# huggingface/optimum-quanto

Hardware: AMD Instinct MI355X
Metric: QLinear GEMM TFLOP/s (bf16 x int8 qbytes_mm) (higher is better)
Workload: dtype bf16; 1 GPU; bf16 x int8 qbytes_mm, per-channel scale, (M,K,N)=(4096,4096,4096); M=4096, K=4096, N=4096, weight_buffers_rotated=1, launch=hipGraph replay of the K steps, parallelism=replicas x1 (no data-path collective)

## Files before the change

### include/quanto_hip.h

```cpp
#ifndef QUANTO_HIP_H_
#define QUANTO_HIP_H_

#include <stddef.h>
#include <stdint.h>

#ifdef __cplusplus
extern "C" {
#endif

#define QUANTO_HIP_ABI_VERSION 1

typedef enum {
  QUANTO_HIP_OK = 0,
  QUANTO_HIP_EINVAL = -1,
  QUANTO_HIP_ENOTSUP = -2,
  QUANTO_HIP_ELAUNCH = -3,
  QUANTO_HIP_EALIGN = -4
} quanto_hip_status;

typedef enum {
  QUANTO_HIP_F32 = 0,
  QUANTO_HIP_F16 = 1,
  QUANTO_HIP_BF16 = 2,
  QUANTO_HIP_I8 = 3,
// ... 59 lines not shown
int64_t quanto_hip_qbits_mm_workspace_size(int64_t M, int64_t N, int64_t K, int bits, int group_size, int dtype,
                                           int kernel);
int quanto_hip_qbits_mm_pick(int64_t M, int64_t N, int64_t K, int bits, int group_size, int dtype);
int quanto_hip_qbits_mm_plan(int64_t M, int64_t N, int64_t K, int bits, int group_size, int dtype, int kernel, int* kernel_out,
                             int64_t* workspace_bytes_out);

int quanto_hip_qbytes_mm(const void* a, const void* b, const void* scales, const void* bias, void* y,
                         int64_t M, int64_t N, int64_t K, int a_dtype, int b_dtype, int out_dtype, int kernel,
                         void* stream);

int quanto_hip_qbytes_mm_multi_ws(const void* a, int count, const void* const* b, const void* const* scales,
                                  const void* const* bias, void* const* y, const int64_t* N, int64_t M, int64_t K, int a_dtype,
                                  int b_dtype, int out_dtype, void* workspace, size_t workspace_bytes, void* stream);
int quanto_hip_qbytes_mm_multi_plan(int count, const int64_t* N, int64_t M, int64_t K, int a_dtype, int b_dtype, int out_dtype,
                                    int* kernel_out, int64_t* workspace_bytes_out);

int quanto_hip_qbytes_mm_ws(const void* a, const void* b, const void* scales, const void* bias, void* y,
                            int64_t M, int64_t N, int64_t K, int a_dtype, int b_dtype, int out_dtype, int kernel,
                            void* workspace, size_t workspace_bytes, void* stream);
int64_t quanto_hip_qbytes_mm_workspace_size(int64_t M, int64_t N, int64_t K, int a_dtype, int b_dtype, int out_dtype, int kernel);
int quanto_hip_qbytes_mm_pick(int64_t M, int64_t N, int64_t K, int a_dtype, int b_dtype, int out_dtype);
int quanto_hip_qbytes_mm_plan(int64_t M, int64_t N, int64_t K, int a_dtype, int b_dtype, int out_dtype, int kernel, int* kernel_out,
                              int64_t* workspace_bytes_out);

int quanto_hip_qbytes_mm_q_ws(const void* a, const void* b, const void* scales, const void* bias, const void* out_scale, void* yq,
                              int64_t M, int64_t N, int64_t K, int a_dtype, int b_dtype, int mid_dtype, int kernel,
                              void* workspace, size_t workspace_bytes, void* stream);
int quanto_hip_qbytes_mm_q_plan(int64_t M, int64_t N, int64_t K, int a_dtype, int b_dtype, int mid_dtype, int kernel, int* kernel_out,
                                int64_t* workspace_bytes_out);

enum quanto_hip_scale_mode { QUANTO_HIP_SCALE_PER_TENSOR = 0, QUANTO_HIP_SCALE_AXIS_FIRST = 1, QUANTO_HIP_SCALE_AXIS_LAST = 2 };
int quanto_hip_quantize_symmetric(const void* base, const void* scale, void* out, int64_t numel, int64_t inner,
                                  int scale_mode, int in_dtype, int out_dtype, void* stream);

int quanto_hip_dequantize_symmetric(const void* q, const void* scale, void* out, int64_t numel, int q_dtype, int out_dtype, void* stream);

int quanto_hip_quantize_affine(const void* base, const void* scale, const void* shift, uint8_t* out, int64_t N, int64_t K,
                               int bits, int group_size, int dtype, int shift_dtype, void* stream);

int quanto_hip_quantize_affine_packed(const void* base, const void* scale, const void* shift, uint8_t* packed, int64_t N, int64_t K,
                                      int bits, int group_size, int dtype, int shift_dtype, void* stream);

int quanto_hip_pack(const uint8_t* unpacked, uint8_t* packed, int64_t rows, int64_t cols, int bits, void* stream);

int quanto_hip_qbits_mm_a8(const void* a, const void* a_scale, const uint8_t* packed, const void* scale, const void* shift, const void* bias, void* y,
                           int64_t M, int64_t N, int64_t K, int bits, int group_size, int a_dtype, int dtype, int shift_dtype, void* workspace,
// ... 57 lines not shown
```

### optimum_quanto_amd/csrc/c_api.hip

```cpp
#include "qh_conv.h"

namespace qh {

static thread_local const char* g_last_kernel = "";
void set_last_kernel(const char* name) { g_last_kernel = name; }

int launch_status() { return hipGetLastError() == hipSuccess ? QUANTO_HIP_OK : QUANTO_HIP_ELAUNCH; }

int unpack_dispatch(const uint8_t*, uint8_t*, int64_t, int, hipStream_t);
int dequantize_qbits_dispatch(const uint8_t*, const void*, const void*, void*, const PackedGeom&, int, bool, hipStream_t);
int qbytes_mm_naive(const void*, const void*, const void*, const void*, void*, int64_t, int64_t, int64_t, int, int, int, hipStream_t);
int qbits_mm_naive(const void*, const uint8_t*, const void*, const void*, const void*, void*, int64_t, const PackedGeom&, int, bool,
                   hipStream_t);
bool qbits_gemv_supported(int64_t, const PackedGeom&, int);
int qbits_mm_gemv(const void*, const uint8_t*, const void*, const void*, const void*, void*, int64_t, const PackedGeom&, int, bool,
                  hipStream_t);
int qbits_mm_gemv_multi(const void*, int, const uint8_t* const*, const void* const*, const void* const*, const void* const*, void* const*,
                        const int64_t*, int64_t, int64_t, int, bool, hipStream_t);
bool qbytes_gemv_supported(int64_t, int64_t, int64_t, int, int, int);
int qbytes_mm_gemv(const void*, const void*, const void*, const void*, void*, int64_t, int64_t, int64_t, int, int, int, hipStream_t);
bool qbytes_mfma_supported(int64_t, int64_t, int64_t, int, int, int);
int qbytes_mm_mfma(const void*, const void*, const void*, const void*, void*, int64_t, int64_t, int64_t, int, int, int, hipStream_t);
bool qbytes_mfma_large_supported(int64_t, int64_t, int64_t, int, int, int);
int qbytes_mm_mfma_large(const void*, const void*, const void*, const void*, void*, int64_t, int64_t, int64_t, int, int, int, void*, size_t, hipStream_t);
size_t qbytes_mfma_large_workspace(int64_t, int64_t, int64_t);
int quantize_symmetric(const void*, const void*, void*, int64_t, int64_t, int, int, int, hipStream_t);
int dequantize_symmetric(const void*, const void*, void*, int64_t, int, int, hipStream_t);
int quantize_affine(const void*, const void*, const void*, void*, int64_t, int64_t, int, int, bool, hipStream_t);
int quantize_affine_packed(const void*, const void*, const void*, void*, int64_t, int64_t, int, int, bool, hipStream_t);
int pack_weights(const uint8_t*, uint8_t*, int64_t, int64_t, int, hipStream_t);
bool qbits_conv2d_supported(const ConvGeom&, const PackedGeom&, int);
int qbits_conv2d_mfma(const void*, const uint8_t*, const void*, const void*, const void*, void*, const ConvGeom&, const PackedGeom&, int, bool, void*, size_t,
                      hipStream_t);
size_t conv2d_workspace(int64_t, int64_t, int64_t);
int qbytes_conv2d_depthwise(const void*, const void*, const void*, const void*, void*, const ConvGeom&, int, int, int, hipStream_t, bool* strip);
size_t conv2d_dense_weight_bytes(int64_t, int64_t);
bool conv2d_rows_eligible(const ConvGeom&);
int qdense_conv2d_rows(const void*, const void*, const void*, void*, const ConvGeom&, int, void*, size_t, hipStream_t);
int qbytes_conv2d_a8_kind(int, int, int);
size_t conv2d_a8_workspace(int64_t, int64_t, int64_t);
int qbytes_conv2d_a8(const void*, const void*, const void*, const void*, const void*, const void*, void*, const ConvGeom&, int, int, int, void*, size_t,
                     hipStream_t, int*);
int qbytes_conv2d_mfma(const void*, const void*, const void*, const void*, void*, const ConvGeom&, int, int, int, void*, size_t, hipStream_t, bool* rows);
int qbytes_mm_gemv_multi(const void*, int, const void* const*, const void* const*, const void* const*, void* const*, const int64_t*, int64_t,
                         int64_t, int, int, hipStream_t);
bool qbytes_skinny_multi_supported(int, const int64_t*, int64_t, int64_t, int, int, int);
size_t qbytes_skinny_multi_workspace(int, const int64_t*, int64_t, int64_t);
int qbytes_mm_skinny_multi(const void*, int, const void* const*, const void* const*, const void* const*, void* const*, const int64_t*, int64_t,
// ... 476 lines not shown
int quanto_hip_qbytes_mm_pick(int64_t M, int64_t N, int64_t K, int a_dtype, int b_dtype, int out_dtype) {
  const int st = check_qbytes(M, N, K, out_dtype);
  return st != QUANTO_HIP_OK ? st : plan_qbytes(M, N, K, a_dtype, b_dtype, out_dtype, QUANTO_HIP_KERNEL_AUTO).kernel;
}

int64_t quanto_hip_qbytes_mm_workspace_size(int64_t M, int64_t N, int64_t K, int a_dtype, int b_dtype, int out_dtype, int kernel) {
  int st = check_qbytes(M, N, K, out_dtype);
  if (st == QUANTO_HIP_OK) st = qbytes_kernel_serves(kernel, M, N, K, a_dtype, b_dtype, out_dtype);
  return st != QUANTO_HIP_OK ? st : plan_qbytes(M, N, K, a_dtype, b_dtype, out_dtype, kernel).workspace;
}

int quanto_hip_qbytes_mm_plan(int64_t M, int64_t N, int64_t K, int a_dtype, int b_dtype, int out_dtype, int kernel, int* kernel_out,
                              int64_t* workspace_bytes_out) {
  if (!kernel_out || !workspace_bytes_out) return QUANTO_HIP_EINVAL;
  int st = check_qbytes(M, N, K, out_dtype);
  if (st == QUANTO_HIP_OK) st = qbytes_kernel_serves(kernel, M, N, K, a_dtype, b_dtype, out_dtype);
  if (st != QUANTO_HIP_OK) return st;
  const Plan p = plan_qbytes(M, N, K, a_dtype, b_dtype, out_dtype, kernel);
  *kernel_out = p.kernel;
  *workspace_bytes_out = p.workspace;
  return QUANTO_HIP_OK;
}

int quanto_hip_qbytes_mm_ws(const void* a, const void* b, const void* scales, const void* bias, void* y, int64_t M, int64_t N, int64_t K,
                            int a_dtype, int b_dtype, int out_dtype, int kernel, void* workspace, size_t workspace_bytes, void* stream_) {
  const int st = check_qbytes(M, N, K, out_dtype);
  if (st != QUANTO_HIP_OK) return st;
  if (M == 0) return QUANTO_HIP_OK;
  if (!a || !b || !scales || !y) return QUANTO_HIP_EINVAL;
  hipStream_t stream = reinterpret_cast<hipStream_t>(stream_);
  if (kernel == QUANTO_HIP_KERNEL_AUTO && (reinterpret_cast<uintptr_t>(a) | reinterpret_cast<uintptr_t>(b)) % 16) kernel = QUANTO_HIP_KERNEL_NAIVE;
  kernel = plan_qbytes(M, N, K, a_dtype, b_dtype, out_dtype, kernel).kernel;
  const bool f32 = a_dtype == QUANTO_HIP_F32 && out_dtype == QUANTO_HIP_F32;
  int r = QUANTO_HIP_EINVAL;
  const char* name = "";
  switch (kernel) {
    case QUANTO_HIP_KERNEL_NAIVE:
      r = qbytes_mm_naive(a, b, scales, bias, y, M, N, K, a_dtype, b_dtype, out_dtype, stream);
      name = "naive";
      break;
    case QUANTO_HIP_KERNEL_GEMV:
      r = f32 ? qbytes_mm_gemv_f32(a, b, scales, bias, y, M, N, K, a_dtype, b_dtype, out_dtype, stream)
              : qbytes_mm_gemv(a, b, scales, bias, y, M, N, K, a_dtype, b_dtype, out_dtype, stream);
      name = f32 ? "gemv_f32" : "gemv";
      break;
    case QUANTO_HIP_KERNEL_SKINNY:
// ... 308 lines not shown
```

### optimum_quanto_amd/csrc/qmm_mfma_large.hip

```cpp
#include <cstdlib>
#include <type_traits>

#include "qmm_large_common.h"

namespace qh {
namespace lt {

#ifdef QH_LT_STAMPS
__device__ unsigned long long g_stamps[256 * 8];
#define QH_LT_STAMP(i) do { if (threadIdx.x == 0) g_stamps[blockIdx.x * 8 + (i)] = __builtin_amdgcn_s_memrealtime(); } while (0)
#else
#define QH_LT_STAMP(i) do { } while (0)
#endif

template <int... Ps, class F>
__device__ __forceinline__ void for_each_slot_impl(std::integer_sequence<int, Ps...>, F&& f) {
  (f(std::integral_constant<int, Ps>{}), ...);
}
template <int R, class F>
__device__ __forceinline__ void for_each_slot(F&& f) {
  for_each_slot_impl(std::make_integer_sequence<int, R>{}, f);
}

template <int DT, int FMT, int BM, int BN, int WM, int WN, int WD = 0>
__global__ void __launch_bounds__(WM * WN * 64, 1) qbytes_mfma_large_kernel(const Args a) {
  constexpr int NWAVES = WM * WN;
  constexpr int MI = BM / WM / 16;
  constexpr int NJ = BN / WN / 16;
  constexpr int STEPS = 2 * MI;
  constexpr int A_BYTES = BM * BK * 2, W_BYTES = WD ? 0 : BN * BK, STAGE_BYTES = A_BYTES + W_BYTES;
  constexpr int APIECES = BM / 8 / NWAVES;
  constexpr int WPIECES = WD ? 0 : BN / 16 / NWAVES;
  constexpr int NPIECES = APIECES + WPIECES;
  constexpr int ND = (NJ * 4 + MI - 1) / MI;
  constexpr int DSTEPS = WD ? 1 : NPIECES % 6 == 0 ? 6 : 3;
  constexpr int PPS = NPIECES / DSTEPS;
  static_assert(WD || (NPIECES % DSTEPS == 0 && PPS <= NJ), "unsupported tile configuration");
  static_assert(STEPS % 4 == 0 && ND <= NJ && APIECES + NJ <= STEPS, "unsupported tile configuration");
  using E = Elem<DT>;
  using T = typename E::T;
  using V8 = typename Mma<DT>::V8;
  extern __shared__ __attribute__((aligned(16))) uint8_t smem[];

  QH_LT_STAMP(0);
  const int tid = threadIdx.x, lane = tid & 63;
  const int wave = __builtin_amdgcn_readfirstlane(tid >> 6);
  const int wm = wave / WN, wn = wave % WN;
  const int M = a.M, N = a.N, K = a.K;
  const int S = a.S;
  const int tile_id = S > 1 ? blockIdx.x / S : blockIdx.x, sp = S > 1 ? blockIdx.x - tile_id * S : 0;
  const int nk = K / BK / S;
  const int kt0 = sp * nk;

  const int tiles_n = (N + BN - 1) / BN, tiles_m = (M + BM - 1) / BM;
  int tm, tn;
  tile_coords(tile_id, tiles_m, tiles_n, a.group_m, tm, tn);
  const int m0 = tm * BM, n0 = tn * BN;

  uint32_t asrc[APIECES], wsrc[WPIECES > 0 ? WPIECES : 1];
#pragma unroll
  for (int j = 0; j < APIECES; ++j) {
    const int R = (j * NWAVES + wave) * 8 + (lane >> 3);
    const int c = (lane & 7) ^ swz_a(R);
    int m = m0 + R;
    m = m < M ? m : M - 1;
    asrc[j] = (uint32_t)(((size_t)m * K + c * 8 + (size_t)kt0 * BK) * 2);
  }
#pragma unroll
  for (int j = 0; j < WPIECES; ++j) {
    const int R = (j * NWAVES + wave) * 16 + (lane >> 2);
    const int c = (lane & 3) ^ swz_w(R);
    int n = n0 + R;
    n = n < N ? n : N - 1;
    wsrc[j] = (uint32_t)((size_t)n * K + c * 16 + (size_t)kt0 * BK);
  }
  const uint32_t lds_base = (uint32_t)(uintptr_t)(lds_ptr_t)smem;
  const uint8_t* xbase = reinterpret_cast<const uint8_t*>(a.x);
  auto issue_piece = [&](int kt, int stage, int piece) {
    const uint32_t stb = __builtin_amdgcn_readfirstlane(lds_base + stage * STAGE_BYTES);
    if (piece < APIECES)
      glds16(xbase + (size_t)kt * (BK * 2), asrc[piece], stb + (piece * NWAVES + wave) * 1024);
    else
      glds16(a.w + (size_t)kt * BK, wsrc[piece - APIECES], stb + A_BYTES + ((piece - APIECES) * NWAVES + wave) * 1024);
  };

  const int ra = wm * (MI * 16) + (lane & 15), rw = wn * (NJ * 16) + (lane & 15);
  int aoff[2];
#pragma unroll
  for (int kk = 0; kk < 2; ++kk) {
    const int chunk = FMT == W_DENSE ? kk * 4 + (lane >> 4) : (lane >> 4) * 2 + kk;
    aoff[kk] = ra * 128 + ((chunk ^ swz_a(ra)) << 4);
  }
  const int boff = A_BYTES + rw * 64 + (((lane >> 4) ^ swz_w(rw)) << 4);

  f32x4 acc[NJ][MI];
#pragma unroll
  for (int j = 0; j < NJ; ++j)
#pragma unroll
    for (int i = 0; i < MI; ++i) acc[j][i] = f32x4{0.f, 0.f, 0.f, 0.f};

  constexpr int RING_BYTES = (WD != 0 ? WD : STAGES) * STAGE_BYTES;
  static_assert(NWAVES * 64 >= 2 * BN, "one table entry per thread");
  FeatureTable<DT, BN> ftab;
  ftab.fetch(a.scale, a.bias, N, n0, tid);

  uint32_t w0[NJ][4], w1[NJ][4];
  V8 xf[4];
  auto as_v8 = [&](const uint32_t(&w)[4]) { return __builtin_bit_cast(V8, make_uint4(w[0], w[1], w[2], w[3])); };
  auto read_x = [&](const uint8_t* st, int i, int kk) -> V8 { return *reinterpret_cast<const V8*>(st + aoff[kk] + i * 2048); };
  using yes = std::integral_constant<bool, true>;

  if constexpr (WD != 0) {
    typedef __attribute__((ext_vector_type(4))) uint32_t u32x4;
    constexpr bool DENSE = FMT == W_DENSE;
    constexpr int WB = DENSE ? 2 : 1;
    constexpr int WLOADS = NJ * WB;
    static_assert(APIECES + WLOADS <= STEPS, "unsupported tile configuration");
    uint32_t wofs[NJ];
#pragma unroll
    for (int j = 0; j < NJ; ++j) {
      int n = n0 + wn * (NJ * 16) + j * 16 + (lane & 15);
      n = n < N ? n : N - 1;
      wofs[j] = (uint32_t)(((size_t)n * K + (size_t)kt0 * BK) * WB + (lane >> 4) * 16);
    }
    constexpr int RING = WD;
    constexpr int GROUP = APIECES + WLOADS;
    constexpr int AHEAD = (RING - 3) * GROUP;
    static_assert(AHEAD <= 63, "vmcnt is a 6-bit counter");
    u32x4 rg[RING][NJ][WB];
    auto load_w = [&](int kt, u32x4 (&dst)[WB], int j) {
      asm volatile("global_load_dwordx4 %0, %1, %2" : "=v"(dst[0]) : "v"(wofs[j]), "s"(a.w + (size_t)kt * (BK * WB)) : "memory");
      if constexpr (DENSE)
        asm volatile("global_load_dwordx4 %0, %1, %2 offset:64" : "=v"(dst[1]) : "v"(wofs[j]), "s"(a.w + (size_t)kt * (BK * WB)) : "memory");
    };
// ... 71 lines not shown
        for (int j = 0; j < NJ; ++j)
#pragma unroll
          for (int b = 0; b < WB; ++b) asm volatile("" : "+v"(rg[(P + 2) % RING][j][b]));
        __builtin_amdgcn_s_barrier();
        asm volatile("" ::: "memory");
      }
    };
    QH_LT_STAMP(3);
    int kt = 0;
    for (; kt + RING < nk; kt += RING)
      for_each_slot<RING>([&](auto p) { tile(p, kt + decltype(p)::value, yes{}, yes{}); });
    for_each_slot<RING>([&](auto p) {
      constexpr int P = decltype(p)::value;
      tile(p, kt + P, std::integral_constant<bool, P == 0>{}, std::integral_constant<bool, P != RING - 1>{});
    });
  } else {
    uint4 raw[NJ];
    auto rawword = [&](int j, int kk, int d) -> uint32_t {
      const uint32_t lo = kk == 0 ? raw[j].x : raw[j].z, hi = kk == 0 ? raw[j].y : raw[j].w;
      return d < 2 ? lo : hi;
    };
    auto read_raw = [&](const uint8_t* st, int j) -> uint4 { return *reinterpret_cast<const uint4*>(st + boff + j * 1024); };

#pragma unroll
    for (int p = 0; p < NPIECES; ++p) issue_piece(0, 0, p);
    if (nk > 1) {
#pragma unroll
      for (int p = 0; p < NPIECES; ++p) issue_piece(1, 1, p);
    }
    asm volatile("s_waitcnt vmcnt(0)" ::: "memory");
    ftab.park(smem + RING_BYTES, tid);
    QH_LT_STAMP(1);
    __builtin_amdgcn_s_barrier();
    asm volatile("" ::: "memory");
    QH_LT_STAMP(2);
#pragma unroll
    for (int j = 0; j < NJ; ++j) raw[j] = read_raw(smem, j);
#pragma unroll
    for (int j = 0; j < NJ; ++j)
#pragma unroll
      for (int d = 0; d < 4; ++d) w0[j][d] = convert_pair<DT, FMT>(rawword(j, 0, d), d & 1);
    xf[0] = read_x(smem, 0, 0);
    xf[1] = read_x(smem, 1, 0);

    const uint8_t* xb[STAGES][2];
    const uint8_t* wb[STAGES];
    uint32_t mdst[STAGES][NPIECES];
#pragma unroll
    for (int t = 0; t < STAGES; ++t) {
      xb[t][0] = smem + t * STAGE_BYTES + aoff[0];
      xb[t][1] = smem + t * STAGE_BYTES + aoff[1];
      wb[t] = smem + t * STAGE_BYTES + boff;
#pragma unroll
      for (int p = 0; p < NPIECES; ++p)
// ... 34 lines not shown
              if (piece < APIECES)
                glds16(xbase + (size_t)(kt + 2) * (BK * 2), asrc[piece], mdst[PF][piece]);
              else
                glds16(a.w + (size_t)(kt + 2) * BK, wsrc[piece - APIECES], mdst[PF][piece]);
            }
          }
          __builtin_amdgcn_sched_barrier(0);
        }
      }
      if (BARRIER) {
        asm volatile("s_waitcnt vmcnt(0)" ::: "memory");
        __builtin_amdgcn_s_barrier();
        asm volatile("" ::: "memory");
      }
    };
    QH_LT_STAMP(3);
    QH_RING3_FOR_EACH_TILE(nk, tile);
  }
  QH_LT_STAMP(4);

  T* yg = reinterpret_cast<T*>(a.y);
  const bool has_bias = a.bias != nullptr;
  const bool full = (m0 + BM <= M) && (n0 + BN <= N) && (N % 8 == 0);
  asm volatile("s_waitcnt lgkmcnt(0)" ::: "memory");
  __builtin_amdgcn_s_barrier();
  asm volatile("" ::: "memory");
  if (S > 1) {
    f32x4* const accf = reinterpret_cast<f32x4*>(acc);
    int* flag = reinterpret_cast<int*>(smem);
    QH_SPLITK_ARRIVE(NJ * MI, NWAVES * 64, a.partials, blockIdx.x, accf, a.counters + tile_id, flag, tid, (void)0, (void)0);
    if (*flag != S - 1) return;
    QH_SPLITK_SUM(NJ * MI, NWAVES * 64, 1, MI, a.partials, tile_id, S, accf, a.counters + tile_id, tid,
                  __syncthreads() );
  }
  constexpr int JP = NJ < 4 ? NJ : 4;
  constexpr int ROWB = JP * 32, LPR = ROWB / 16;
  constexpr int RH = MI >= 8 ? 2 : 1, MIH = MI / RH;
  uint8_t* park = smem + wave * (MI * 16 * ROWB);
  const T* tab = reinterpret_cast<const T*>(smem + RING_BYTES);
#pragma unroll
  for (int p = 0; p < NJ / JP; ++p) {
    float sc[JP][4], bv[JP][4];
#pragma unroll
    for (int jj = 0; jj < JP; ++jj) {
      const int nl = wn * (NJ * 16) + (p * JP + jj) * 16 + (lane >> 4) * 4;
      T sct[4], bvt[4];
      *reinterpret_cast<uint2*>(sct) = *reinterpret_cast<const uint2*>(tab + nl);
      *reinterpret_cast<uint2*>(bvt) = *reinterpret_cast<const uint2*>(tab + BN + nl);
#pragma unroll
      for (int r = 0; r < 4; ++r) {
        sc[jj][r] = E::to_f32(sct[r]);
        bv[jj][r] = E::to_f32(bvt[r]);
      }
    }
#pragma unroll
    for (int h = 0; h < RH; ++h) {
#pragma unroll
      for (int jj = 0; jj < JP; ++jj) {
        const int j = p * JP + jj;
#pragma unroll
        for (int i = h * MIH; i < (h + 1) * MIH; ++i) {
          T out[4];
#pragma unroll
          for (int r = 0; r < 4; ++r) {
            float v = acc[j][i][r] * sc[jj][r];
            asm volatile("" : "+v"(v));
            if (has_bias) v = E::to_f32(E::from_f32(v)) + bv[jj][r];
            out[r] = E::from_f32(v);
          }
          const int row = i * 16 + (lane & 15);
          const int chunk = (jj * 4 + (lane >> 4)) ^ ((row & (LPR - 1)) << 1);
          *reinterpret_cast<uint2*>(park + row * ROWB + chunk * 8) = *reinterpret_cast<const uint2*>(out);
        }
      }
      asm volatile("s_waitcnt lgkmcnt(0)" ::: "memory");
#pragma unroll
      for (int t = h * (MIH * 16 * LPR / 64); t < (h + 1) * (MIH * 16 * LPR / 64); ++t) {
        const int row = t * (64 / LPR) + lane / LPR;
        const int c16 = lane % LPR;
        const uint4 v = *reinterpret_cast<const uint4*>(park + row * ROWB + (((c16 * 2) ^ ((row & (LPR - 1)) << 1)) * 8));
        const int m = m0 + wm * (MI * 16) + row;
        const int n = n0 + wn * (NJ * 16) + p * (JP * 16) + c16 * 8;
        if (full) {
          typedef __attribute__((ext_vector_type(4))) uint32_t u32x4;
          __builtin_nontemporal_store(__builtin_bit_cast(u32x4, v), reinterpret_cast<u32x4*>(yg + (size_t)m * N + n));
        } else if (m < M) {
          const T* e = reinterpret_cast<const T*>(&v);
#pragma unroll
          for (int r = 0; r < 8; ++r)
            if (n + r < N) yg[(size_t)m * N + n + r] = e[r];
        }
      }
    }
    asm volatile("s_waitcnt lgkmcnt(0)" ::: "memory");
  }
  QH_LT_STAMP(5);
  asm volatile("s_waitcnt vmcnt(0)" ::: "memory");
  QH_LT_STAMP(6);
}

enum { CFG_256_8W = 0, CFG_256_4W = 1, CFG_128_4W = 2, CFG_256_1X8 = 3 };

template <int DT, int FMT, int BM, int BN, int WM, int WN, int WD = 0>
static int launch_cfg(const Args& a, hipStream_t stream) {
  constexpr int lds0 = WD != 0 ? WD * (BM * BK * 2) : STAGES * (BM * BK * 2 + BN * BK);
  const int pad = env_int("QUANTO_HIP_LARGE_LDS_PAD", 0);
  const int lds = lds0 + 2 * BN * 2 + pad;
  static_assert(lds0 >= BM * BN * 2, "the epilogue parks the output tile in the stage memory");
  const int tiles_m = (a.M + BM - 1) / BM, tiles_n = (a.N + BN - 1) / BN, tiles = tiles_m * tiles_n;
  Args b = a;
  b.group_m = raster_group_m(tiles, tiles_m, BM, BN);
  (void)hipFuncSetAttribute(reinterpret_cast<const void*>(&qbytes_mfma_large_kernel<DT, FMT, BM, BN, WM, WN, WD>),
                            hipFuncAttributeMaxDynamicSharedMemorySize, lds);
  hipLaunchKernelGGL((qbytes_mfma_large_kernel<DT, FMT, BM, BN, WM, WN, WD>), dim3(tiles * b.S), dim3(WM * WN * 64), lds, stream, b);
  return launch_status();
}

template <int DT, int FMT>
static int launch(const Args& a, int cfg, hipStream_t stream) {
  if (cfg == CFG_128_4W) {
    const int wd = env_int("QUANTO_HIP_LARGE_WD", 1);
    const int nk = a.K / BK / a.S;
    const int tiles = ((a.M + 127) / 128) * ((a.N + 127) / 128);
    if ((wd & 1) && (tiles * a.S <= 256 || (wd & 4)) && nk % 4 == 0 && nk >= 8) return launch_cfg<DT, FMT, 128, 128, 1, 4, 4>(a, stream);
    return launch_cfg<DT, FMT, 128, 128, 1, 4>(a, stream);
  }
#ifdef QH_LT_EXPERIMENTS
  if (cfg == CFG_256_4W) return launch_cfg<DT, FMT, 256, 256, 2, 2>(a, stream);
#else
  if (cfg == CFG_256_4W) return QUANTO_HIP_ENOTSUP;
#endif
  if constexpr (FMT == W_F8E4M3FNUZ) {
    return launch_cfg<DT, FMT, 256, 256, 1, 8>(a, stream);
  } else {
    if (cfg == CFG_256_1X8) return launch_cfg<DT, FMT, 256, 256, 1, 8>(a, stream);
    return launch_cfg<DT, FMT, 256, 256, 2, 4>(a, stream);
  }
}

}

bool qbytes_mfma_large_supported(int64_t M, int64_t N, int64_t K, int a_dtype, int b_dtype, int out_dtype) {
  const bool bd = b_dtype == QUANTO_HIP_I8 || b_dtype == QUANTO_HIP_F8_E4M3FN || b_dtype == QUANTO_HIP_F8_E5M2 || b_dtype == QUANTO_HIP_F8_E4M3FNUZ;
  return bd && a_dtype == out_dtype && (out_dtype == QUANTO_HIP_BF16 || out_dtype == QUANTO_HIP_F16) && K % lt::BK == 0 &&
         K >= 2 * lt::BK && M >= 1 && M * K < (1ll << 30) && N * K < (1ll << 31) && M < (1 << 30) && N < (1 << 30);
}

static int large_split(int64_t M, int64_t N, int64_t K) {
  const int forced = env_int("QUANTO_HIP_LARGE_SPLIT", 0);
  const int64_t tiles256 = ((M + 255) / 256) * ((N + 255) / 256), tiles128 = ((M + 127) / 128) * ((N + 127) / 128);
  int s = 1;
  if (tiles128 <= 128 && (K / lt::BK) % 8 == 0 && K / lt::BK >= 16) s = 2;
  if (tiles128 <= 32 && (K / lt::BK) % 16 == 0 && K / lt::BK >= 32) s = 4;
  if (forced > 0 && tiles128 <= 512 && (K / lt::BK) % forced == 0 && K / lt::BK / forced >= 2) s = forced;
  (void)tiles256;
  if (!ws_counters_fit(tiles128)) s = 1;
  return s;
}
size_t qbytes_mfma_large_workspace(int64_t M, int64_t N, int64_t K) {
  const int S = large_split(M, N, K);
  if (S == 1) return 0;
  return QUANTO_HIP_WS_COUNTER_BYTES + (size_t)(((M + 127) / 128) * ((N + 127) / 128)) * S * (128 * 128 * 4);
}

bool dense_mm_wd_supported(int64_t M, int64_t N, int64_t K, int dtype) {
  const int on = env_int("QUANTO_HIP_DENSE_WD", 1);
  const int64_t tiles128 = ((M + 127) / 128) * ((N + 127) / 128);
  return on && (dtype == QUANTO_HIP_BF16 || dtype == QUANTO_HIP_F16) && K % (4 * lt::BK) == 0 && K >= 8 * lt::BK && M >= 1 &&
         tiles128 <= 256 && M * K < (1ll << 30) && N * K < (1ll << 30);
}

int dense_mm_wd(const void* x, const void* w, const void* bias, void* y, int64_t M, int64_t N, int64_t K, int dtype, hipStream_t stream) {
  if (!dense_mm_wd_supported(M, N, K, dtype)) return QUANTO_HIP_ENOTSUP;
  if ((reinterpret_cast<uintptr_t>(x) | reinterpret_cast<uintptr_t>(w)) % 16) return QUANTO_HIP_EALIGN;
  lt::Args a{x, reinterpret_cast<const uint8_t*>(w), nullptr, bias, y, (int)M, (int)N, (int)K, 1, 1, nullptr, nullptr};
  if (dtype == QUANTO_HIP_BF16) return lt::launch_cfg<QUANTO_HIP_BF16, lt::W_DENSE, 128, 128, 1, 4, 4>(a, stream);
  return lt::launch_cfg<QUANTO_HIP_F16, lt::W_DENSE, 128, 128, 1, 4, 4>(a, stream);
}

int qbytes_mm_mfma_large(const void* x, const void* w, const void* s, const void* bias, void* y, int64_t M, int64_t N, int64_t K, int a_dtype,
                      int b_dtype, int out_dtype, void* workspace, size_t workspace_bytes, hipStream_t stream) {
  if (!qbytes_mfma_large_supported(M, N, K, a_dtype, b_dtype, out_dtype)) return QUANTO_HIP_ENOTSUP;
  int split = large_split(M, N, K);
  if (split > 1 && !ws_holds(workspace, workspace_bytes, qbytes_mfma_large_workspace(M, N, K))) split = 1;
  const int forced = env_int("QUANTO_HIP_LARGE_CFG", -1);
  const int64_t tiles128 = ((M + 127) / 128) * ((N + 127) / 128);
  const int cfg256 = b_dtype == QUANTO_HIP_F8_E4M3FNUZ ? lt::CFG_256_1X8 : lt::CFG_256_8W;
  const int cfg = forced >= 0 ? forced : (tiles128 > 512 ? cfg256 : lt::CFG_128_4W);
  if (cfg != lt::CFG_128_4W) split = 1;
  if ((reinterpret_cast<uintptr_t>(x) | reinterpret_cast<uintptr_t>(w)) % 16) return QUANTO_HIP_EALIGN;
  lt::Args a{x, reinterpret_cast<const uint8_t*>(w), s, bias, y, (int)M, (int)N, (int)K, 1, split, reinterpret_cast<int*>(workspace),
             split > 1 ? ws_partials(workspace) : nullptr};
#define QH_CASE(DT, FMT) return lt::launch<DT, FMT>(a, cfg, stream)
  if (out_dtype == QUANTO_HIP_BF16) {
    if (b_dtype == QUANTO_HIP_I8) QH_CASE(QUANTO_HIP_BF16, lt::W_I8);
    if (b_dtype == QUANTO_HIP_F8_E4M3FN) QH_CASE(QUANTO_HIP_BF16, lt::W_F8E4M3);
    if (b_dtype == QUANTO_HIP_F8_E4M3FNUZ) QH_CASE(QUANTO_HIP_BF16, lt::W_F8E4M3FNUZ);
    QH_CASE(QUANTO_HIP_BF16, lt::W_F8E5M2);
  }
  if (b_dtype == QUANTO_HIP_I8) QH_CASE(QUANTO_HIP_F16, lt::W_I8);
  if (b_dtype == QUANTO_HIP_F8_E4M3FN) QH_CASE(QUANTO_HIP_F16, lt::W_F8E4M3);
  if (b_dtype == QUANTO_HIP_F8_E4M3FNUZ) QH_CASE(QUANTO_HIP_F16, lt::W_F8E4M3FNUZ);
  QH_CASE(QUANTO_HIP_F16, lt::W_F8E5M2);
#undef QH_CASE
}

}
```

### optimum_quanto_amd/library/hip.py

```python
import ctypes
import os
import re

import torch

from .extension import NativeLibrary, register_extension

__all__ = ["quanto_hip", "QuantoHipError"]

_PKG_DIR = os.path.dirname(os.path.dirname(os.path.abspath(__file__)))

F32, F16, BF16, I8, U8, F8_E4M3FN, F8_E5M2, F8_E4M3FNUZ = range(8)
WS_COUNTER_BYTES = 4096
def _c_atoi(v: str) -> int:
    m = re.match(r"\s*([+-]?\d+)", v or "")
    return int(m.group(1)) if m else 0


_EXPERIMENT = _c_atoi(os.environ.get("QUANTO_HIP_EXPERIMENT", "0")) != 0
KERNEL_AUTO, KERNEL_NAIVE, KERNEL_GEMV, KERNEL_MFMA, KERNEL_MFMA_LARGE, KERNEL_SKINNY, KERNEL_NATIVE8, KERNEL_DEQUANT_MFMA, KERNEL_MFMA_FUSED4, KERNEL_MMV, KERNEL_MFMA_LARGE4 = range(11)
KERNELS = {"auto": KERNEL_AUTO, "naive": KERNEL_NAIVE, "gemv": KERNEL_GEMV, "mfma": KERNEL_MFMA, "mfma_large": KERNEL_MFMA_LARGE, "skinny": KERNEL_SKINNY,
           "mfma_native8": KERNEL_NATIVE8, "dequant_mfma": KERNEL_DEQUANT_MFMA, "mfma_fused4": KERNEL_MFMA_FUSED4, "mmv": KERNEL_MMV, "mfma_large4": KERNEL_MFMA_LARGE4}

_DTYPES = {
# ... 60 lines not shown
    "quanto_hip_abi_version": (_ci, None),
    "quanto_hip_status_string": (ctypes.c_char_p, [_ci]),
    "quanto_hip_last_kernel": (ctypes.c_char_p, None),
    "quanto_hip_stream_capture_id": (_i64, [_vp]),
    "quanto_hip_unpack": (_ci, [_vp, _vp, _i64, _ci, _vp]),
    "quanto_hip_dequantize_qbits": (_ci, [_vp] * 4 + [_i64] * 2 + [_ci] * 4 + [_vp]),
    "quanto_hip_qbits_mm": (_ci, [_vp] * 6 + [_i64] * 3 + [_ci] * 5 + [_vp, _sz, _vp]),
    "quanto_hip_qbits_mm_multi": (_ci, [_vp, _ci] + [_pvp] * 5 + [_pi64, _i64, _i64] + [_ci] * 4 + [_vp]),
    "quanto_hip_qbits_mm_multi_ws": (_ci, [_vp, _ci] + [_pvp] * 5 + [_pi64, _i64, _i64] + [_ci] * 4 + [_vp, _sz, _vp]),
    "quanto_hip_qbits_mm_multi_plan": (_ci, [_ci, _pi64, _i64, _i64] + [_ci] * 3 + [_pci, _pi64]),
    "quanto_hip_qbytes_mm_multi_ws": (_ci, [_vp, _ci] + [_pvp] * 4 + [_pi64, _i64, _i64] + [_ci] * 3 + [_vp, _sz, _vp]),
    "quanto_hip_qbytes_mm_multi_plan": (_ci, [_ci, _pi64, _i64, _i64] + [_ci] * 3 + [_pci, _pi64]),
    "quanto_hip_qbits_mm_workspace_size": (_i64, [_i64] * 3 + [_ci] * 4),
    "quanto_hip_qbits_mm_plan": (_ci, [_i64] * 3 + [_ci] * 4 + [_pci, _pi64]),
    "quanto_hip_qbits_mm_pick": (_ci, [_i64] * 3 + [_ci] * 3),
    "quanto_hip_qbits_mm_a8": (_ci, [_vp] * 7 + [_i64] * 3 + [_ci] * 5 + [_vp, _sz, _vp]),
    "quanto_hip_qbits_mm_a8_workspace_size": (_i64, [_i64] * 3 + [_ci] * 4),
    "quanto_hip_qbits_mm_a8_q": (_ci, [_vp] * 8 + [_i64] * 3 + [_ci] * 5 + [_vp, _sz, _vp]),
    "quanto_hip_qbytes_mm": (_ci, [_vp] * 5 + [_i64] * 3 + [_ci] * 4 + [_vp]),
    "quanto_hip_qbytes_mm_ws": (_ci, [_vp] * 5 + [_i64] * 3 + [_ci] * 4 + [_vp, _sz, _vp]),
    "quanto_hip_qbytes_mm_workspace_size": (_i64, [_i64] * 3 + [_ci] * 4),
    "quanto_hip_qbytes_mm_plan": (_ci, [_i64] * 3 + [_ci] * 4 + [_pci, _pi64]),
    "quanto_hip_qbytes_mm_pick": (_ci, [_i64] * 3 + [_ci] * 3),
    "quanto_hip_qbytes_mm_q_ws": (_ci, [_vp] * 6 + [_i64] * 3 + [_ci] * 4 + [_vp, _sz, _vp]),
    "quanto_hip_qbytes_mm_q_plan": (_ci, [_i64] * 3 + [_ci] * 4 + [_pci, _pi64]),
    "quanto_hip_qbytes_bmm": (_ci, [_vp] * 4 + [_i64] * 9 + [_ci, _vp]),
    "quanto_hip_layer_norm_q": (_ci, [_vp] * 5 + [_i64] * 3 + [ctypes.c_float, _ci, _ci, _vp]),
    "quanto_hip_layer_norm_q_supported": (_ci, [_i64] * 2 + [_ci] * 2),
    "quanto_hip_quantize_symmetric": (_ci, [_vp] * 3 + [_i64] * 2 + [_ci] * 3 + [_vp]),
    "quanto_hip_dequantize_symmetric": (_ci, [_vp] * 3 + [_i64] + [_ci] * 2 + [_vp]),
    "quanto_hip_quantize_affine": (_ci, [_vp] * 4 + [_i64] * 2 + [_ci] * 4 + [_vp]),
    "quanto_hip_quantize_affine_packed": (_ci, [_vp] * 4 + [_i64] * 2 + [_ci] * 4 + [_vp]),
    "quanto_hip_pack": (_ci, [_vp, _vp, _i64, _i64, _ci, _vp]),
    "quanto_hip_qbytes_conv2d": (_ci, [_vp] * 5 + [_i64] * 9 + [_ci] * 9 + [_vp, _sz, _vp]),
    "quanto_hip_qbytes_conv2d_depthwise": (_ci, [_vp] * 5 + [_i64] * 9 + [_ci] * 9 + [_vp]),
    "quanto_hip_qbytes_conv2d_a8": (_ci, [_vp] * 6 + [_i64] * 9 + [_ci] * 9 + [_vp, _sz, _vp]),
    "quanto_hip_qbytes_conv2d_a8_workspace_size": (_i64, [_i64] * 9 + [_ci] * 9),
    "quanto_hip_qbytes_conv2d_a8_q": (_ci, [_vp] * 7 + [_i64] * 9 + [_ci] * 9 + [_vp, _sz, _vp]),
    "quanto_hip_conv2d_workspace_size": (_i64, [_i64] * 5),
    "quanto_hip_qbits_conv2d_workspace_size": (_i64, [_i64] * 5),
    "quanto_hip_qbits_conv2d_workspace_size_geom": (_i64, [_i64] * 8 + [_ci] * 2),
    "quanto_hip_qbits_conv2d": (_ci, [_vp] * 6 + [_i64] * 9 + [_ci] * 10 + [_vp, _sz, _vp]),
}


class _Bindings:
# ... 666 lines not shown
```

Baseline: 1418 TFLOP/s.

## Add persistent 256-tile MFMA GEMM that prefetches next tile during epilogue

Adds a persistent form of the 256x256 LDS-weight MFMA kernel, launched with a grid sized to the CU count. Each workgroup loops over output tiles and issues the first two K-stage loads of its next tile before running the current tile's epilogue, so loads overlap the epilogue. The epilogue now parks a quarter of the output tile at a time in the last stage, and the scale/bias table is double-buffered. This reduces epilogue and launch-tail bubbles, at the cost of a more serialised epilogue and extra LDS. It is enabled by default for the int8 256-tile config when K<=4096.

```diff
diff --git a/include/quanto_hip.h b/include/quanto_hip.h
--- a/include/quanto_hip.h
+++ b/include/quanto_hip.h
@@ -105,6 +105,8 @@
 int quanto_hip_qbytes_mm_pick(int64_t M, int64_t N, int64_t K, int a_dtype, int b_dtype, int out_dtype);
 int quanto_hip_qbytes_mm_plan(int64_t M, int64_t N, int64_t K, int a_dtype, int b_dtype, int out_dtype, int kernel, int* kernel_out,
                               int64_t* workspace_bytes_out);
+int quanto_hip_qbytes_mm_large_persist_plan(int64_t M, int64_t N, int64_t K, int a_dtype, int b_dtype, int out_dtype, int compute_units,
+                                            int* workgroups_out);
 
 int quanto_hip_qbytes_mm_q_ws(const void* a, const void* b, const void* scales, const void* bias, const void* out_scale, void* yq,
                               int64_t M, int64_t N, int64_t K, int a_dtype, int b_dtype, int mid_dtype, int kernel,
diff --git a/optimum_quanto_amd/csrc/c_api.hip b/optimum_quanto_amd/csrc/c_api.hip
--- a/optimum_quanto_amd/csrc/c_api.hip
+++ b/optimum_quanto_amd/csrc/c_api.hip
@@ -24,6 +24,7 @@
 bool qbytes_mfma_large_supported(int64_t, int64_t, int64_t, int, int, int);
 int qbytes_mm_mfma_large(const void*, const void*, const void*, const void*, void*, int64_t, int64_t, int64_t, int, int, int, void*, size_t, hipStream_t);
 size_t qbytes_mfma_large_workspace(int64_t, int64_t, int64_t);
+int qbytes_mfma_large_persist_workgroups(int64_t, int64_t, int64_t, int, int);
 int quantize_symmetric(const void*, const void*, void*, int64_t, int64_t, int, int, int, hipStream_t);
 int dequantize_symmetric(const void*, const void*, void*, int64_t, int, int, hipStream_t);
 int quantize_affine(const void*, const void*, const void*, void*, int64_t, int64_t, int, int, bool, hipStream_t);
@@ -546,6 +547,16 @@
   return QUANTO_HIP_OK;
 }
 
+int quanto_hip_qbytes_mm_large_persist_plan(int64_t M, int64_t N, int64_t K, int a_dtype, int b_dtype, int out_dtype, int compute_units,
+                                            int* workgroups_out) {
+  if (!workgroups_out || compute_units < 0) return QUANTO_HIP_EINVAL;
+  int st = check_qbytes(M, N, K, out_dtype);
+  if (st == QUANTO_HIP_OK) st = qbytes_kernel_serves(QUANTO_HIP_KERNEL_MFMA_LARGE, M, N, K, a_dtype, b_dtype, out_dtype);
+  if (st != QUANTO_HIP_OK) return st;
+  *workgroups_out = qbytes_mfma_large_persist_workgroups(M, N, K, b_dtype, compute_units);
+  return QUANTO_HIP_OK;
+}
+
 int quanto_hip_qbytes_mm_ws(const void* a, const void* b, const void* scales, const void* bias, void* y, int64_t M, int64_t N, int64_t K,
                             int a_dtype, int b_dtype, int out_dtype, int kernel, void* workspace, size_t workspace_bytes, void* stream_) {
   const int st = check_qbytes(M, N, K, out_dtype);
diff --git a/optimum_quanto_amd/csrc/qmm_mfma_large.hip b/optimum_quanto_amd/csrc/qmm_mfma_large.hip
--- a/optimum_quanto_amd/csrc/qmm_mfma_large.hip
+++ b/optimum_quanto_amd/csrc/qmm_mfma_large.hip
@@ -22,8 +22,12 @@
   for_each_slot_impl(std::make_integer_sequence<int, R>{}, f);
 }
 
-template <int DT, int FMT, int BM, int BN, int WM, int WN, int WD = 0>
+constexpr int PERSISTENT = -1;
+template <int DT, int FMT, int BM, int BN, int WM, int WN, int WDP = 0>
 __global__ void __launch_bounds__(WM * WN * 64, 1) qbytes_mfma_large_kernel(const Args a) {
+  constexpr bool PERSIST = WDP == PERSISTENT;
+  constexpr int WD = PERSIST ? 0 : WDP;
+  static_assert(!PERSIST || (WD == 0 && BM == 256 && BN == 256), "the persistent form exists for the LDS-weights 256-tiles");
   constexpr int NWAVES = WM * WN;
   constexpr int MI = BM / WM / 16;
   constexpr int NJ = BN / WN / 16;
@@ -47,33 +51,38 @@
   const int wave = __builtin_amdgcn_readfirstlane(tid >> 6);
   const int wm = wave / WN, wn = wave % WN;
   const int M = a.M, N = a.N, K = a.K;
-  const int S = a.S;
-  const int tile_id = S > 1 ? blockIdx.x / S : blockIdx.x, sp = S > 1 ? blockIdx.x - tile_id * S : 0;
+  const int S = PERSIST ? 1 : a.S;
+  int tile_id = S > 1 ? blockIdx.x / S : blockIdx.x;
+  const int sp = S > 1 ? blockIdx.x - tile_id * S : 0;
   const int nk = K / BK / S;
   const int kt0 = sp * nk;
 
   const int tiles_n = (N + BN - 1) / BN, tiles_m = (M + BM - 1) / BM;
-  int tm, tn;
-  tile_coords(tile_id, tiles_m, tiles_n, a.group_m, tm, tn);
-  const int m0 = tm * BM, n0 = tn * BN;
-
+  int m0, n0;
   uint32_t asrc[APIECES], wsrc[WPIECES > 0 ? WPIECES : 1];
-#pragma unroll
-  for (int j = 0; j < APIECES; ++j) {
-    const int R = (j * NWAVES + wave) * 8 + (lane >> 3);
-    const int c = (lane & 7) ^ swz_a(R);
-    int m = m0 + R;
-    m = m < M ? m : M - 1;
-    asrc[j] = (uint32_t)(((size_t)m * K + c * 8 + (size_t)kt0 * BK) * 2);
-  }
-#pragma unroll
-  for (int j = 0; j < WPIECES; ++j) {
-    const int R = (j * NWAVES + wave) * 16 + (lane >> 2);
-    const int c = (lane & 3) ^ swz_w(R);
-    int n = n0 + R;
-    n = n < N ? n : N - 1;
-    wsrc[j] = (uint32_t)((size_t)n * K + c * 16 + (size_t)kt0 * BK);
-  }
+  auto tile_sources = [&](int id, int ln) {
+    int tm, tn;
+    tile_coords(id, tiles_m, tiles_n, a.group_m, tm, tn);
+    m0 = tm * BM;
+    n0 = tn * BN;
+#pragma unroll
+    for (int j = 0; j < APIECES; ++j) {
+      const int R = (j * NWAVES + wave) * 8 + (ln >> 3);
+      const int c = (ln & 7) ^ swz_a(R);
+      int m = m0 + R;
+      m = m < M ? m : M - 1;
+      asrc[j] = (uint32_t)(((size_t)m * K + c * 8 + (size_t)kt0 * BK) * 2);
+    }
+#pragma unroll
+    for (int j = 0; j < WPIECES; ++j) {
+      const int R = (j * NWAVES + wave) * 16 + (ln >> 2);
+      const int c = (ln & 3) ^ swz_w(R);
+      int n = n0 + R;
+      n = n < N ? n : N - 1;
+      wsrc[j] = (uint32_t)((size_t)n * K + c * 16 + (size_t)kt0 * BK);
+    }
+  };
+  tile_sources(tile_id, lane);
   const uint32_t lds_base = (uint32_t)(uintptr_t)(lds_ptr_t)smem;
   const uint8_t* xbase = reinterpret_cast<const uint8_t*>(a.x);
   auto issue_piece = [&](int kt, int stage, int piece) {
@@ -103,6 +112,7 @@
   static_assert(NWAVES * 64 >= 2 * BN, "one table entry per thread");
   FeatureTable<DT, BN> ftab;
   ftab.fetch(a.scale, a.bias, N, n0, tid);
+  uint8_t* tab_slot = smem + RING_BYTES;
 
   uint32_t w0[NJ][4], w1[NJ][4];
   V8 xf[4];
@@ -110,6 +120,7 @@
   auto read_x = [&](const uint8_t* st, int i, int kk) -> V8 { return *reinterpret_cast<const V8*>(st + aoff[kk] + i * 2048); };
   using yes = std::integral_constant<bool, true>;
 
+  for (bool first_tile = true;; first_tile = false) {
   if constexpr (WD != 0) {
     typedef __attribute__((ext_vector_type(4))) uint32_t u32x4;
     constexpr bool DENSE = FMT == W_DENSE;
@@ -227,14 +238,16 @@
     };
     auto read_raw = [&](const uint8_t* st, int j) -> uint4 { return *reinterpret_cast<const uint4*>(st + boff + j * 1024); };
 
-#pragma unroll
-    for (int p = 0; p < NPIECES; ++p) issue_piece(0, 0, p);
-    if (nk > 1) {
-#pragma unroll
-      for (int p = 0; p < NPIECES; ++p) issue_piece(1, 1, p);
+    if (first_tile) {
+#pragma unroll
+      for (int p = 0; p < NPIECES; ++p) issue_piece(0, 0, p);
+      if (nk > 1) {
+#pragma unroll
+        for (int p = 0; p < NPIECES; ++p) issue_piece(1, 1, p);
+      }
     }
     asm volatile("s_waitcnt vmcnt(0)" ::: "memory");
-    ftab.park(smem + RING_BYTES, tid);
+    ftab.park(tab_slot, tid);
     QH_LT_STAMP(1);
     __builtin_amdgcn_s_barrier();
     asm volatile("" ::: "memory");
@@ -315,9 +328,25 @@
   T* yg = reinterpret_cast<T*>(a.y);
   const bool has_bias = a.bias != nullptr;
   const bool full = (m0 + BM <= M) && (n0 + BN <= N) && (N % 8 == 0);
+  const int em0 = m0, en0 = n0;
   asm volatile("s_waitcnt lgkmcnt(0)" ::: "memory");
   __builtin_amdgcn_s_barrier();
   asm volatile("" ::: "memory");
+  int elane = lane;
+  bool more = false;
+  if constexpr (PERSIST) {
+    asm volatile("" : "+v"(elane));
+    tile_id += gridDim.x;
+    more = tile_id < tiles_m * tiles_n;
+    if (more) {
+      tile_sources(tile_id, elane);
+      ftab.fetch(a.scale, a.bias, N, n0, tid);
+#pragma unroll
+      for (int p = 0; p < NPIECES; ++p) issue_piece(0, 0, p);
+#pragma unroll
+      for (int p = 0; p < NPIECES; ++p) issue_piece(1, 1, p);
+    }
+  }
   if (S > 1) {
     f32x4* const accf = reinterpret_cast<f32x4*>(acc);
     int* flag = reinterpret_cast<int*>(smem);
@@ -328,15 +357,16 @@
   }
   constexpr int JP = NJ < 4 ? NJ : 4;
   constexpr int ROWB = JP * 32, LPR = ROWB / 16;
-  constexpr int RH = MI >= 8 ? 2 : 1, MIH = MI / RH;
-  uint8_t* park = smem + wave * (MI * 16 * ROWB);
-  const T* tab = reinterpret_cast<const T*>(smem + RING_BYTES);
+  constexpr int RH = PERSIST ? 4 : MI >= 8 ? 2 : 1, MIH = MI / RH;
+  static_assert(!PERSIST || (NJ <= 4 && MI % 4 == 0 && NWAVES * MIH * 16 * ROWB <= STAGE_BYTES), "a quarter of the output tile is parked in one stage");
+  uint8_t* park = PERSIST ? smem + 2 * STAGE_BYTES + wave * (MIH * 16 * ROWB) : smem + wave * (MI * 16 * ROWB);
+  const T* tab = reinterpret_cast<const T*>(tab_slot);
 #pragma unroll
   for (int p = 0; p < NJ / JP; ++p) {
     float sc[JP][4], bv[JP][4];
 #pragma unroll
     for (int jj = 0; jj < JP; ++jj) {
-      const int nl = wn * (NJ * 16) + (p * JP + jj) * 16 + (lane >> 4) * 4;
+      const int nl = wn * (NJ * 16) + (p * JP + jj) * 16 + (elane >> 4) * 4;
       T sct[4], bvt[4];
       *reinterpret_cast<uint2*>(sct) = *reinterpret_cast<const uint2*>(tab + nl);
       *reinterpret_cast<uint2*>(bvt) = *reinterpret_cast<const uint2*>(tab + BN + nl);
@@ -348,6 +378,7 @@
     }
 #pragma unroll
     for (int h = 0; h < RH; ++h) {
+      const int prow0 = PERSIST ? h * (MIH * 16) : 0;
 #pragma unroll
       for (int jj = 0; jj < JP; ++jj) {
         const int j = p * JP + jj;
@@ -361,19 +392,19 @@
             if (has_bias) v = E::to_f32(E::from_f32(v)) + bv[jj][r];
             out[r] = E::from_f32(v);
           }
-          const int row = i * 16 + (lane & 15);
-          const int chunk = (jj * 4 + (lane >> 4)) ^ ((row & (LPR - 1)) << 1);
-          *reinterpret_cast<uint2*>(park + row * ROWB + chunk * 8) = *reinterpret_cast<const uint2*>(out);
+          const int row = i * 16 + (elane & 15);
+          const int chunk = (jj * 4 + (elane >> 4)) ^ ((row & (LPR - 1)) << 1);
+          *reinterpret_cast<uint2*>(park + (row - prow0) * ROWB + chunk * 8) = *reinterpret_cast<const uint2*>(out);
         }
       }
       asm volatile("s_waitcnt lgkmcnt(0)" ::: "memory");
 #pragma unroll
       for (int t = h * (MIH * 16 * LPR / 64); t < (h + 1) * (MIH * 16 * LPR / 64); ++t) {
-        const int row = t * (64 / LPR) + lane / LPR;
-        const int c16 = lane % LPR;
-        const uint4 v = *reinterpret_cast<const uint4*>(park + row * ROWB + (((c16 * 2) ^ ((row & (LPR - 1)) << 1)) * 8));
-        const int m = m0 + wm * (MI * 16) + row;
-        const int n = n0 + wn * (NJ * 16) + p * (JP * 16) + c16 * 8;
+        const int row = t * (64 / LPR) + elane / LPR;
+        const int c16 = elane % LPR;
+        const uint4 v = *reinterpret_cast<const uint4*>(park + (row - prow0) * ROWB + (((c16 * 2) ^ ((row & (LPR - 1)) << 1)) * 8));
+        const int m = em0 + wm * (MI * 16) + row;
+        const int n = en0 + wn * (NJ * 16) + p * (JP * 16) + c16 * 8;
         if (full) {
           typedef __attribute__((ext_vector_type(4))) uint32_t u32x4;
           __builtin_nontemporal_store(__builtin_bit_cast(u32x4, v), reinterpret_cast<u32x4*>(yg + (size_t)m * N + n));
@@ -387,6 +418,13 @@
     }
     asm volatile("s_waitcnt lgkmcnt(0)" ::: "memory");
   }
+  if (!PERSIST || !more) break;
+#pragma unroll
+  for (int j = 0; j < NJ; ++j)
+#pragma unroll
+    for (int i = 0; i < MI; ++i) acc[j][i] = f32x4{0.f, 0.f, 0.f, 0.f};
+  tab_slot = smem + RING_BYTES + (tab_slot == smem + RING_BYTES ? FeatureTable<DT, BN>::BYTES : 0);
+  }
   QH_LT_STAMP(5);
   asm volatile("s_waitcnt vmcnt(0)" ::: "memory");
   QH_LT_STAMP(6);
@@ -394,23 +432,28 @@
 
 enum { CFG_256_8W = 0, CFG_256_4W = 1, CFG_128_4W = 2, CFG_256_1X8 = 3 };
 
-template <int DT, int FMT, int BM, int BN, int WM, int WN, int WD = 0>
-static int launch_cfg(const Args& a, hipStream_t stream) {
+template <int DT, int FMT, int BM, int BN, int WM, int WN, int WDP = 0>
+static int launch_cfg(const Args& a, hipStream_t stream, int persist_wgs = 0) {
+  constexpr bool PERSIST = WDP == PERSISTENT;
+  constexpr int WD = PERSIST ? 0 : WDP;
   constexpr int lds0 = WD != 0 ? WD * (BM * BK * 2) : STAGES * (BM * BK * 2 + BN * BK);
   const int pad = env_int("QUANTO_HIP_LARGE_LDS_PAD", 0);
-  const int lds = lds0 + 2 * BN * 2 + pad;
-  static_assert(lds0 >= BM * BN * 2, "the epilogue parks the output tile in the stage memory");
+  const int lds = lds0 + (PERSIST ? 2 : 1) * 2 * BN * 2 + pad;
+  static_assert(PERSIST || lds0 >= BM * BN * 2, "the epilogue parks the output tile in the stage memory");
+  static_assert(!PERSIST || lds0 / STAGES >= BM * BN * 2 / 4, "the persistent epilogue parks a quarter of the output tile in the last stage");
   const int tiles_m = (a.M + BM - 1) / BM, tiles_n = (a.N + BN - 1) / BN, tiles = tiles_m * tiles_n;
   Args b = a;
   b.group_m = raster_group_m(tiles, tiles_m, BM, BN);
-  (void)hipFuncSetAttribute(reinterpret_cast<const void*>(&qbytes_mfma_large_kernel<DT, FMT, BM, BN, WM, WN, WD>),
+  if (PERSIST) b.S = 1;
+  const int grid = PERSIST ? (persist_wgs < tiles ? persist_wgs : tiles) : tiles * b.S;
+  (void)hipFuncSetAttribute(reinterpret_cast<const void*>(&qbytes_mfma_large_kernel<DT, FMT, BM, BN, WM, WN, WDP>),
                             hipFuncAttributeMaxDynamicSharedMemorySize, lds);
-  hipLaunchKernelGGL((qbytes_mfma_large_kernel<DT, FMT, BM, BN, WM, WN, WD>), dim3(tiles * b.S), dim3(WM * WN * 64), lds, stream, b);
+  hipLaunchKernelGGL((qbytes_mfma_large_kernel<DT, FMT, BM, BN, WM, WN, WDP>), dim3(grid), dim3(WM * WN * 64), lds, stream, b);
   return launch_status();
 }
 
 template <int DT, int FMT>
-static int launch(const Args& a, int cfg, hipStream_t stream) {
+static int launch(const Args& a, int cfg, hipStream_t stream, int persist_wgs = 0) {
   if (cfg == CFG_128_4W) {
     const int wd = env_int("QUANTO_HIP_LARGE_WD", 1);
     const int nk = a.K / BK / a.S;
@@ -427,6 +470,7 @@
     return launch_cfg<DT, FMT, 256, 256, 1, 8>(a, stream);
   } else {
     if (cfg == CFG_256_1X8) return launch_cfg<DT, FMT, 256, 256, 1, 8>(a, stream);
+    if (persist_wgs > 0) return launch_cfg<DT, FMT, 256, 256, 2, 4, PERSISTENT>(a, stream, persist_wgs);
     return launch_cfg<DT, FMT, 256, 256, 2, 4>(a, stream);
   }
 }
@@ -471,20 +515,49 @@
   return lt::launch_cfg<QUANTO_HIP_F16, lt::W_DENSE, 128, 128, 1, 4, 4>(a, stream);
 }
 
+static int large_cfg(int64_t M, int64_t N, int b_dtype) {
+  const int forced = env_int("QUANTO_HIP_LARGE_CFG", -1);
+  const int64_t tiles128 = ((M + 127) / 128) * ((N + 127) / 128);
+  const int cfg256 = b_dtype == QUANTO_HIP_F8_E4M3FNUZ ? lt::CFG_256_1X8 : lt::CFG_256_8W;
+  return forced >= 0 ? forced : (tiles128 > 512 ? cfg256 : lt::CFG_128_4W);
+}
+
+int qbytes_mfma_large_persist_workgroups(int64_t M, int64_t N, int64_t K, int b_dtype, int cus) {
+  const int mode = env_int("QUANTO_HIP_LARGE_PERSIST", 1);
+  const int cfg = large_cfg(M, N, b_dtype);
+  if (mode <= 0 || cfg != lt::CFG_256_8W || b_dtype == QUANTO_HIP_F8_E4M3FNUZ) return 0;
+  int g = cus / 8 * 8;
+  const int wgs = env_int("QUANTO_HIP_LARGE_PERSIST_WGS", 0);
+  if (wgs >= 8) g = wgs / 8 * 8;
+  if (g < 8) return 0;
+  const int64_t tiles256 = ((M + 255) / 256) * ((N + 255) / 256);
+  return mode >= 2 || (tiles256 > g && K <= 4096) ? g : 0;
+}
+
+static int device_cus() {
+  static int cached[64];
+  int dev = 0;
+  if (hipGetDevice(&dev) != hipSuccess || dev < 0 || dev >= 64) return 0;
+  int n = __atomic_load_n(&cached[dev], __ATOMIC_RELAXED);
+  if (n == 0) {
+    if (hipDeviceGetAttribute(&n, hipDeviceAttributeMultiprocessorCount, dev) != hipSuccess || n < 0) n = 0;
+    __atomic_store_n(&cached[dev], n, __ATOMIC_RELAXED);
+  }
+  return n;
+}
+
 int qbytes_mm_mfma_large(const void* x, const void* w, const void* s, const void* bias, void* y, int64_t M, int64_t N, int64_t K, int a_dtype,
                       int b_dtype, int out_dtype, void* workspace, size_t workspace_bytes, hipStream_t stream) {
   if (!qbytes_mfma_large_supported(M, N, K, a_dtype, b_dtype, out_dtype)) return QUANTO_HIP_ENOTSUP;
   int split = large_split(M, N, K);
   if (split > 1 && !ws_holds(workspace, workspace_bytes, qbytes_mfma_large_workspace(M, N, K))) split = 1;
-  const int forced = env_int("QUANTO_HIP_LARGE_CFG", -1);
-  const int64_t tiles128 = ((M + 127) / 128) * ((N + 127) / 128);
-  const int cfg256 = b_dtype == QUANTO_HIP_F8_E4M3FNUZ ? lt::CFG_256_1X8 : lt::CFG_256_8W;
-  const int cfg = forced >= 0 ? forced : (tiles128 > 512 ? cfg256 : lt::CFG_128_4W);
+  const int cfg = large_cfg(M, N, b_dtype);
   if (cfg != lt::CFG_128_4W) split = 1;
   if ((reinterpret_cast<uintptr_t>(x) | reinterpret_cast<uintptr_t>(w)) % 16) return QUANTO_HIP_EALIGN;
+  const int persist_wgs = cfg == lt::CFG_256_8W ? qbytes_mfma_large_persist_workgroups(M, N, K, b_dtype, device_cus()) : 0;
   lt::Args a{x, reinterpret_cast<const uint8_t*>(w), s, bias, y, (int)M, (int)N, (int)K, 1, split, reinterpret_cast<int*>(workspace),
              split > 1 ? ws_partials(workspace) : nullptr};
-#define QH_CASE(DT, FMT) return lt::launch<DT, FMT>(a, cfg, stream)
+#define QH_CASE(DT, FMT) return lt::launch<DT, FMT>(a, cfg, stream, persist_wgs)
   if (out_dtype == QUANTO_HIP_BF16) {
     if (b_dtype == QUANTO_HIP_I8) QH_CASE(QUANTO_HIP_BF16, lt::W_I8);
     if (b_dtype == QUANTO_HIP_F8_E4M3FN) QH_CASE(QUANTO_HIP_BF16, lt::W_F8E4M3);
diff --git a/optimum_quanto_amd/library/hip.py b/optimum_quanto_amd/library/hip.py
--- a/optimum_quanto_amd/library/hip.py
+++ b/optimum_quanto_amd/library/hip.py
@@ -106,6 +106,7 @@
     "quanto_hip_qbytes_mm_workspace_size": (_i64, [_i64] * 3 + [_ci] * 4),
     "quanto_hip_qbytes_mm_plan": (_ci, [_i64] * 3 + [_ci] * 4 + [_pci, _pi64]),
     "quanto_hip_qbytes_mm_pick": (_ci, [_i64] * 3 + [_ci] * 3),
+    "quanto_hip_qbytes_mm_large_persist_plan": (_ci, [_i64] * 3 + [_ci] * 4 + [_pci]),
     "quanto_hip_qbytes_mm_q_ws": (_ci, [_vp] * 6 + [_i64] * 3 + [_ci] * 4 + [_vp, _sz, _vp]),
     "quanto_hip_qbytes_mm_q_plan": (_ci, [_i64] * 3 + [_ci] * 4 + [_pci, _pi64]),
     "quanto_hip_qbytes_bmm": (_ci, [_vp] * 4 + [_i64] * 9 + [_ci, _vp]),
```

After: 1409 TFLOP/s. About the same (-0.6%).
